# menickname/waafle

Hardware: AMD Instinct MI355X
Metric: contigs scored/sec + k2 clade-pair evals/sec at 1/2/4/8 MI355X vs CPU ref (higher is better)
Workload: dtype f64

## Files before the change

waafle_amd/csrc/wf_device.h:

```cpp
#pragma once
#include "wf_internal.h"

#include "waafle_hip.h"
#include "wf_lanes.h"

namespace wf {

namespace {


constexpr uint64_t kKeyPad = ~0ull;

#include "wf_stamps.h"
constexpr int kLocVirtual = 0xFFFF;

__device__ __forceinline__ void note_ppot(const KArgs& K, int c, int iteration, int Pp) {
  if (!K.ppot || Pp < 2) return;
  const uint64_t old = (uint64_t)K.ppot[c];
  if (iteration > (int)(old >> 40))
    K.ppot[c] = (int64_t)(((uint64_t)iteration << 40) | ((old & ((1ull << 40) - 1ull)) + (uint64_t)Pp));
}

__device__ __forceinline__ bool e2_no_option(const KArgs& K, int c, int iteration, int64_t pair_evals, bool root,
                                             int32_t* pend) {
  const int lane = threadIdx.x & 63;
  if (!root && iteration + 1 <= kMaxIter) {
    if (lane == 0) {
      pend[c] = 2;
      K.pair_evals[c] = pair_evals;
    }
    return true;
  }
  if (lane == 0) {
    K.iters[c] = (int16_t)min(root ? iteration : iteration + 1, 32767);
    K.pair_evals[c] = pair_evals;
    K.status[c] = root ? 0 : WF_E_RUNAWAY;
  }
  return false;
}

struct Ctl {
  int A, A1, npow, S_n, P, Gu, Pp;
  int overflow, status, cnt, cnt2, p_unk, root_present, all_ignored;
  int n_in, all_ok, all_same, best_ok, best_dir, best_c1p, best_c2p;
  int lca1, lca2, res_kind, lca_out;
  int cls_cnt[5], cls_off[5];
  double best_r, best_crit;
  long long best_k;
  int64_t need;
  double red_r[kWaves];
  long long red_k[kWaves];
  int red_i[kWaves];
  int red_j[kWaves];
};

__device__ __forceinline__ int lane_id() { return threadIdx.x & 63; }
__device__ __forceinline__ int wave_id() { return threadIdx.x >> 6; }

struct Arena {
  char* base;
  int64_t cap;
  int64_t used;
  template <class T>
  __device__ __forceinline__ T* take(int64_t count) {
    int64_t off = (used + 15) & ~int64_t(15);
    used = off + count * (int64_t)sizeof(T);
    return reinterpret_cast<T*>(base + off);
  }
  __device__ __forceinline__ bool fits() const { return used <= cap; }
};

__device__ __forceinline__ uint64_t dbits(double x) { return (uint64_t)__double_as_longlong(x); }

template <class T>
__device__ __forceinline__ const T& kernarg_fresh(const T& arg) {
#ifdef __HIP_DEVICE_COMPILE__
  uint64_t a = reinterpret_cast<uint64_t>(__builtin_amdgcn_kernarg_segment_ptr());
  asm volatile("" : "+s"(a));
  return *reinterpret_cast<const __attribute__((address_space(4))) T*>(a);
#else
  return arg;
#endif
}


template <int NT>
__device__ __forceinline__ int block_scan(int v, int* total, Ctl& ctl) {
  const int lane = lane_id(), w = wave_id();
  int x = v;
#pragma unroll
  for (int d = 1; d < 64; d <<= 1) {
    int y = __shfl_up(x, d, 64);
    if (lane >= d) x += y;
  }
  if (lane == 63) ctl.red_i[w] = x;
  __syncthreads();
  int base = 0, tot = 0;
#pragma unroll
  for (int i = 0; i < NT / 64; ++i) {
    int t = ctl.red_i[i];
    base += (i < w) ? t : 0;
    tot += t;
  }
  __syncthreads();
  *total = tot;
  return base + x - v;
}

template <int NT>
__device__ __forceinline__ void block_scan2(int v1, int v2, int* p1, int* p2, int* t1, int* t2, Ctl& ctl) {
  const int lane = lane_id(), w = wave_id();
  int x = v1, y = v2;
#pragma unroll
  for (int d = 1; d < 64; d <<= 1) {
    int a = __shfl_up(x, d, 64), b = __shfl_up(y, d, 64);
    if (lane >= d) { x += a; y += b; }
  }
  if (lane == 63) { ctl.red_i[w] = x; ctl.red_j[w] = y; }
  __syncthreads();
  int b1 = 0, b2 = 0, s1 = 0, s2 = 0;
#pragma unroll
  for (int i = 0; i < NT / 64; ++i) {
    int a = ctl.red_i[i], b = ctl.red_j[i];
    if (i < w) { b1 += a; b2 += b; }
    s1 += a;
    s2 += b;
  }
  __syncthreads();
  *p1 = b1 + x - v1;
  *p2 = b2 + y - v2;
  *t1 = s1;
  *t2 = s2;
}

__device__ __forceinline__ bool better(double r2, long long k2, double r, long long k) {
  return k2 >= 0 && (k < 0 || r2 > r || (r2 == r && k2 > k));
}

template <int NT>
__device__ __forceinline__ void block_argmax(double& r, long long& k, Ctl& ctl) {
#pragma unroll
  for (int off = 32; off > 0; off >>= 1) {
    double r2 = __shfl_xor(r, off, 64);
    long long k2 = __shfl_xor(k, off, 64);
    if (better(r2, k2, r, k)) { r = r2; k = k2; }
  }
  if (lane_id() == 0) { ctl.red_r[wave_id()] = r; ctl.red_k[wave_id()] = k; }
  __syncthreads();
  if (threadIdx.x == 0) {
    double br = ctl.red_r[0];
    long long bk = ctl.red_k[0];
    for (int i = 1; i < NT / 64; ++i)
      if (better(ctl.red_r[i], ctl.red_k[i], br, bk)) { br = ctl.red_r[i]; bk = ctl.red_k[i]; }
    ctl.best_r = br;
    ctl.best_k = bk;
  }
  __syncthreads();
  r = ctl.best_r;
  k = ctl.best_k;
}

template <int NT, class T>
__device__ __forceinline__ void bitonic_sort(T* keys, int n) {
  for (int k = 2; k <= n; k <<= 1) {
// ... 1674 lines not shown
```

waafle_amd/csrc/wf_fast.hip:

```cpp
#include <algorithm>
#include <cstdlib>

#include "wf_device.h"
#include "wf_lanes.h"

namespace wf {

namespace {

constexpr int kSlotBits = 9;
constexpr int kCladeShift = 15;
constexpr uint32_t kSlotMask = (1u << kSlotBits) - 1;
constexpr int kLoc0 = 64;
constexpr int kLut0 = 256;
constexpr int kAnn0 = 64;
constexpr int kRuns0 = 64;
constexpr int kMultiAtt0 = 32;
constexpr int kRunsL0 = 32;
constexpr int kMultiAttL0 = 16;
constexpr int kXcds = 8;
constexpr int kRollWaves = 4;
constexpr int kPot0 = 64;
constexpr int kS0 = 640;

// ... 446 lines not shown
    b_ok = lane_bcast(b_ok, 0); b_dir = lane_bcast(b_dir, 0);
    b_c1p = lane_bcast(b_c1p, 0); b_c2p = lane_bcast(b_c2p, 0);
    bcrit = lane_bcast(bcrit, 0);
    wave_sync();
    int n_in = 0;
    bool all_ok = true, all_same = true;
    uint64_t b1 = 0, b2 = 0;
    for (int i = 0; i + 1 < Pp; ++i) {
      const uint64_t mi = pmask[i];
      for (int j = i + 1 + lane; j < Pp; j += 64) {
        if ((mi | pmask[j]) != full) continue;
        const double r = pair_rank(C, i, j, Gu);
        if (!((br - r) <= P.range)) continue;
        const OptEval e = eval_two_call(K, C, Pn, i, j, F.best_syn(), nullptr);
        ++n_in;
        all_ok = all_ok && e.ok;
        all_same = all_same && e.same;
        b1 |= 1ull << e.c1p;
        b2 |= 1ull << e.c2p;
      }
    }
    n_in = wave_sum_dpp(n_in);
    b1 = wave_or_dpp(b1);
    b2 = wave_or_dpp(b2);
    all_ok = __ballot(!all_ok) == 0ull;
    all_same = __ballot(!all_same) == 0ull;
    int kind;
    if (n_in == 0) kind = (P.dis2 == 0) ? 3 : (P.dis2 == 1 ? 0 : 4);
    else if (n_in == 1 || P.dis2 == 0) kind = 1;
    else if (P.dis2 == 1) kind = 0;
    else kind = (all_ok && all_same) ? 2 : 0;
    if (kind == 4) {
      if (lane == 0) K.status[c] = WF_E_BADINPUT;
      return kDecDone;
    }
    bool have_ok = false;
    int lca1 = -1, lca2v = -1;
    const int m1 = __popcll(b1), m2 = __popcll(b2);
    if (kind == 2) {
      const bool in1 = lane < Pp && ((b1 >> lane) & 1ull), in2 = lane < Pp && ((b2 >> lane) & 1ull);
      lca1 = wave_lca(K, in1 ? F.cl()[lane] : -1);
      lca2v = wave_lca(K, in2 ? F.cl()[lane] : -1);
      bool keep = true;
      if (!P.allow_lca) {
        const int nl = lca2(K, lca1, lca2v);
        keep = !(nl == lca1 || nl == lca2v);
      }
      have_ok = keep;
      if (have_ok) {
        if (in1) K.meld[C.mbase + __popcll(b1 & lanes_below())] = F.cl()[lane];
        if (in2) K.meld[C.mbase + m1 + __popcll(b2 & lanes_below())] = F.cl()[lane];
      }
    } else if (kind == 1) {
      have_ok = b_ok != 0;
    } else if (kind == 3) {
      have_ok = true;
    }
    if (have_ok) {
      if (lane < G) K.syn[l0 + lane] = F.best_syn()[lane];
      if (lane == 0) {
        K.call[c] = WF_CALL_LGT;
        K.crit[c] = bcrit;
        K.rank[c] = br;
        K.dir[c] = (int8_t)b_dir;
        K.c1[c] = (kind == 2) ? lca1 : F.cl()[b_c1p];
        K.c2[c] = (kind == 2) ? lca2v : F.cl()[b_c2p];
        K.nm1[c] = (kind == 2) ? m1 : 0;
        K.nm2[c] = (kind == 2) ? m2 : 0;
        K.iters[c] = (int16_t)iteration;
        K.pair_evals[c] = pair_evals;
      }
      return kDecDone;
    }
  }
  return (Pn == 0 || root) ? kDecStop : kDecRaise;
}

template <int CAP, bool FULL, bool ROLL = false>
__global__ __launch_bounds__(64, FULL ? 2 : (ROLL ? kRollWaves : 4)) void k_wave(const SArgs S_arg, int64_t* ccnt, int64_t* cleaves, int32_t* pend,
                                             const int32_t* list, int n_list, const int64_t* n_dev, int rollup,
                                             int start_level_arg) {
  static_assert(!(FULL && ROLL), "the roll-up passes are first-form launches");
  const int start_level = ROLL ? start_level_arg : 0;
  if (n_dev) n_list = (int)*n_dev;
  if (S_arg.wq && (int)blockIdx.x >= n_list) return;
  extern __shared__ __attribute__((aligned(16))) char smem[];
  WaveSmem<CAP, FULL>& F = *reinterpret_cast<WaveSmem<CAP, FULL>*>(smem);
  const int lane = threadIdx.x;
  const bool xmap = gridDim.x % kXcds == 0;
  const int xb = (int)gridDim.x / kXcds, xj = (int)blockIdx.x / kXcds, xx = (int)blockIdx.x % kXcds;
  for (int it = 0;; ++it) {
    int ci;
    if (S_arg.wq) {
      unsigned long long q = 0;
      if (lane == 0) q = atomicAdd(S_arg.wq, 1ull);
      ci = __builtin_amdgcn_readfirstlane((int)q);
    } else {
      ci = xmap ? (it * kXcds + xx) * xb + xj : (int)blockIdx.x + it * (int)gridDim.x;
    }
    if (ci >= n_list) break;
    const int c = list ? list[ci] : ci;
    WLAP_MARK();
    const SArgs& S = kernarg_fresh<SArgs>(S_arg);
    const KArgs& K = S.k;
    const DevParams& P = K.p;
    const int nsys = K.n_sys;
    const bool ann_on = !ROLL && nsys > 0;
    if (FULL && P.weak == 2) continue;
    const int64_t h0 = K.hit_off[c], h1 = K.hit_off[c + 1];
    constexpr int kHB = 4;
    int r_qlo[kHB], r_qhi[kHB], r_hs[kHB], r_cl[kHB];
    double r_scv[kHB], r_sc[kHB];
    uint32_t r_m[kHB];
    auto load_round = [&](int64_t hq) {
#pragma unroll
      for (int b = 0; b < kHB; ++b) {
        const int64_t h = hq + 64 * b + lane;
        r_qlo[b] = 0; r_qhi[b] = 0; r_hs[b] = 0; r_cl[b] = 0;
        r_scv[b] = 0.0; r_sc[b] = 0.0; r_m[b] = 0u;
        if (h < h1) {
          r_scv[b] = K.scov[h];
          r_qlo[b] = K.qlo[h];
          r_qhi[b] = K.qhi[h];
          if (P.stranded) r_hs[b] = K.hstrand[h];
          r_cl[b] = K.taxon[h];
          r_sc[b] = K.score[h];
          if (ann_on) r_m[b] = K.sysmask[h];
        }
      }
    };
    load_round(h0);
    const int64_t l0 = K.loc_off[c];
    const int G = (int)(K.loc_off[c + 1] - l0);
    const int Gs = min(G, kLoc0);
    int nl1 = 0;
    int my_lo = 0, my_hi = -1;
    if (lane < Gs) {
      const int a = K.lstart[l0 + lane], b = K.lend[l0 + lane];
      const int len = max(a, b) - min(a, b) + 1;
      my_lo = min(a, b);
      my_hi = max(a, b);
      F.lo[lane] = my_lo;
      F.len[lane] = len;
      F.st[lane] = K.lstrand[l0 + lane];
      if (len < kNpyBuf) nl1 = S.lut_off[len + 1] - S.lut_off[len];
      F.nl1[lane] = (int16_t)nl1;
    }
    const int prev_hi = __shfl_up(my_hi, 1, 64);
    const bool ordered = G <= kLoc0 && P.min_overlap > 0.0 &&
                         __ballot(lane >= 1 && lane < Gs && my_lo <= prev_hi) == 0ull;
    int lut_total;
    const int lb = wave_excl_scan(nl1, &lut_total);
    F.lbase[lane] = (int16_t)min(lb, 32767);
    const int nann = Gs * nsys;
    F.abest()[lane] = 0ull;
    F.ahit()[lane] = -1;
    const bool long_locus = __ballot(lane < Gs && F.len[lane] > 65535) != 0ull;
    bool staged = G > kLoc0 || lut_total > kLut0 || nann > kAnn0 || long_locus;
    wave_sync();
    bool lut_ready = false;
    auto load_lut = [&]() {
      for (int i = lane; i < lut_total; i += 64) {
        int g = 0;
        for (int b = 32; b > 0; b >>= 1)
          if (g + b < Gs && F.lbase[g + b] <= i) g += b;
        F.lut[i] = pack_leaf(S.lut[S.lut_off[F.len[g]] + (i - F.lbase[g])]);
      }
      wave_sync();
      lut_ready = true;
    };

    WLAP(0);
    int n_att = 0;
    long long nl_sum = 0;
    for (int64_t hq = h0; hq < h1; hq += 64 * kHB) {
      if (hq != h0) load_round(hq);
    for (int bq = 0; bq < kHB && hq + 64 * bq < h1; ++bq) {
      const int64_t hb = hq + 64 * bq;
      const int64_t h = hb + lane;
      int qlo = r_qlo[0], qhi = r_qhi[0], hs = r_hs[0], clade = r_cl[0];
      double scv = r_scv[0], sc = r_sc[0];
      uint32_t m = r_m[0];
      int n = 0;
      uint64_t am = 0ull;
#pragma unroll
      for (int b = 1; b < kHB; ++b)
        if (bq == b) {
          qlo = r_qlo[b]; qhi = r_qhi[b]; hs = r_hs[b]; clade = r_cl[b];
          scv = r_scv[b]; sc = r_sc[b]; m = r_m[b];
        }
      if (ordered && h < h1 && scv >= P.min_scov) {
        int g = 0;
#pragma unroll
        for (int k = 32; k > 0; k >>= 1) {
          const int i = min(g + k, Gs) - 1;
          if (g + k <= Gs && F.lo[i] + F.len[i] - 1 < qlo) g += k;
        }
        for (; g < Gs; ++g) {
          const int lo = F.lo[g], len = F.len[g];
          if (lo > qhi) break;
          if (attaches(P, qlo, qhi, hs, lo, len, F.st[g])) {
            ++n;
            nl_sum += len < kNpyBuf ? F.nl1[g] : leaves_for(S, len);
            am |= 1ull << g;
          }
        }
        if (ROLL && n > 0) clade = S.anc[clade];
      } else if (!ordered && h < h1 && scv >= P.min_scov) {
        for (int g = 0; g < G; ++g) {
          int lo, len, st;
          if (g < kLoc0) {
            lo = F.lo[g]; len = F.len[g]; st = F.st[g];
          } else {
            const int a = K.lstart[l0 + g], b = K.lend[l0 + g];
            lo = min(a, b); len = max(a, b) - lo + 1; st = K.lstrand[l0 + g];
          }
          if (attaches(P, qlo, qhi, hs, lo, len, st)) {
            ++n;
            nl_sum += (g < kLoc0 && len < kNpyBuf) ? F.nl1[g] : leaves_for(S, len);
            if (g < kLoc0) am |= 1ull << g;
          }
        }
        if (ROLL && n > 0) clade = S.anc[clade];
      }
      int total;
      const int o = wave_excl_scan(n, &total);
      if (!staged && n > 0 && n_att + o + n <= CAP) {
        if (!ROLL)
          for (int j = 0; j < P.jump; ++j) clade = K.parent[clade];
        const bool ann = m != 0 && sc >= P.annot_ref;
// ... 730 lines not shown
            S.dump_cg[base + t] = cg_of(F, t);
            S.dump_mean[base + t] = out_v(t);
          }
        }
        if (lane == 0) {
          S.dump_first[slot] = (int)(base < INT32_MAX ? base : INT32_MAX);
          S.dump_first[slot + 1] = (int)(base + n_out < INT32_MAX ? base + n_out : INT32_MAX);
          S.dump_list[2 * slot] = compact ? 1 : 0;
          S.dump_list[2 * slot + 1] = dumped ? c : -1;
          if (compact) S.dump_um[slot] = um | (rootp ? (1ull << 63) : 0ull);
        }
        staged = true;
        WSTAT(21, 1);
        WLAP(9);
        break;
      }
      WLAP(9);
      if (staged || outcome == 2) break;
      const int Gu = __popcll(um);
      wave_sync();
      int dec = -1;
      if constexpr (FULL) dec = wave_two(S, F, c, h0, l0, G, ns, um, Gu, iteration, pair_evals);
      if (dec < 0) {
        staged = true;
        break;
      }
      if (dec == kDecDone) break;
      if (dec == kDecRaise && iteration + 1 <= kMaxIter) {
        if (!rollup) {
          staged = true;
          seed = iteration == 1;
          if (lane == 0) K.pair_evals[c] = pair_evals;
          break;
        }
        wave_sync();
        continue;
      }
      if (lane == 0) {
        K.iters[c] = (int16_t)min(dec == kDecRaise ? iteration + 1 : iteration, 32767);
        K.pair_evals[c] = pair_evals;
        K.status[c] = dec == kDecRaise ? WF_E_RUNAWAY : 0;
      }
      break;
    }
    if (lane == 0) {
      ccnt[c] = staged ? n_att : 0;
      cleaves[c] = staged ? nl_sum : 0;
      const int pd = staged ? (dumped ? 3 : (seed ? 2 : 1)) : 0;
      pend[c] = pd;
      if (pd == 1 && S.fail_ctr) atomicAdd(S.fail_ctr, 1ull);
    }
    WSTAT(22, staged ? 1 : 0);
    wave_sync();
    WLAP(10);
  }
}

template <int CAP, bool FULL, bool ROLL = false>
int blocks_per_cu() {
  static const int n = [] {
    const int bytes = (int)sizeof(WaveSmem<CAP, FULL>);
    (void)hipFuncSetAttribute(reinterpret_cast<const void*>(&k_wave<CAP, FULL, ROLL>),
                              hipFuncAttributeMaxDynamicSharedMemorySize, bytes);
    int b = 0;
    if (hipOccupancyMaxActiveBlocksPerMultiprocessor(&b, reinterpret_cast<const void*>(&k_wave<CAP, FULL, ROLL>), 64,
                                                     bytes) != hipSuccess || b < 1)
      b = 1;
    return b;
  }();
  return n;
}

template <int CAP, bool FULL, bool ROLL = false>
hipError_t launch_cap(const SArgs& sa, int64_t* ccnt, int64_t* cleaves, int32_t* pend, const int32_t* list,
                      int n_list, const int64_t* n_dev, int cus, int rollup, hipStream_t s, int start_level = 0) {
  const unsigned grid = (unsigned)std::max<int64_t>(1, std::min<int64_t>(n_list, (int64_t)cus * blocks_per_cu<CAP, FULL, ROLL>()));
  hipLaunchKernelGGL((k_wave<CAP, FULL, ROLL>), dim3(grid), dim3(64), sizeof(WaveSmem<CAP, FULL>), s, sa, ccnt, cleaves, pend,
                     list, n_list, n_dev, rollup, start_level);
  return hipGetLastError();
}

}

WF_STAMP_READER(fast, g_wstamps, 48)

hipError_t launch_fast(const SArgs& sa, int64_t* ccnt, int64_t* cleaves, int32_t* pend, int max_hits, int cus,
                       hipStream_t s) {
  const int N = sa.k.n_contigs;
  if (max_hits <= 224) return launch_cap<224, false>(sa, ccnt, cleaves, pend, nullptr, N, nullptr, cus, 0, s);
  return max_hits <= 256 ? launch_cap<256, false>(sa, ccnt, cleaves, pend, nullptr, N, nullptr, cus, 0, s)
                         : launch_cap<512, false>(sa, ccnt, cleaves, pend, nullptr, N, nullptr, cus, 0, s);
}

hipError_t launch_fast_list(const SArgs& sa, int64_t* ccnt, int64_t* cleaves, int32_t* pend, const int32_t* list,
                            const int64_t* n_dev, int max_hits, int cus, hipStream_t s) {
  const int N = sa.k.n_contigs;
  if (max_hits <= 224) return launch_cap<224, false>(sa, ccnt, cleaves, pend, list, N, n_dev, cus, 0, s);
  return max_hits <= 256 ? launch_cap<256, false>(sa, ccnt, cleaves, pend, list, N, n_dev, cus, 0, s)
                         : launch_cap<512, false>(sa, ccnt, cleaves, pend, list, N, n_dev, cus, 0, s);
}

hipError_t launch_level(const SArgs& sa, int64_t* ccnt, int64_t* cleaves, int32_t* pend, const int32_t* list,
                        const int64_t* n_dev, int level, int max_hits, int cus, hipStream_t s) {
  const int N = sa.k.n_contigs;
  if (max_hits <= 224) return launch_cap<224, false, true>(sa, ccnt, cleaves, pend, list, N, n_dev, cus, 0, s, level);
  return max_hits <= 256 ? launch_cap<256, false, true>(sa, ccnt, cleaves, pend, list, N, n_dev, cus, 0, s, level)
                         : launch_cap<512, false, true>(sa, ccnt, cleaves, pend, list, N, n_dev, cus, 0, s, level);
}

hipError_t launch_full(const SArgs& sa, int64_t* ccnt, int64_t* cleaves, int32_t* pend, const int32_t* list,
                       const int64_t* n_dev, int max_hits, int cus, bool rollup, hipStream_t s) {
  const int N = sa.k.n_contigs;
  return max_hits <= 256 ? launch_cap<256, true>(sa, ccnt, cleaves, pend, list, N, n_dev, cus, rollup, s)
                         : launch_cap<512, true>(sa, ccnt, cleaves, pend, list, N, n_dev, cus, rollup, s);
}

}
```

waafle_amd/csrc/wf_stamps.h:

```cpp
#pragma once
#ifdef WF_STAMPS
#ifndef WF_STAMPS_ROLL
#define WF_STAMPS_ROLL 0
#endif
#define WF_STAMPS_ONLY(...) __VA_ARGS__
#define WF_STAMP_READER(tag, arr, n)                                                          \
  extern "C" int wf_stamps_read_##tag(unsigned long long* out, int m) {                       \
    if (m > (n)) m = (n);                                                                     \
    return hipMemcpyFromSymbol(out, HIP_SYMBOL(arr), sizeof(unsigned long long) * m) == hipSuccess ? 0 : -2; \
  }                                                                                           \
  extern "C" int wf_stamps_reset_##tag(void) {                                                \
    unsigned long long z[n] = {0};                                                            \
    return hipMemcpyToSymbol(HIP_SYMBOL(arr), z, sizeof z) == hipSuccess ? 0 : -2;            \
  }
__device__ unsigned long long g_stamps[32];
__shared__ unsigned long long g_tlast;
#define STAMP_INIT() do { if (threadIdx.x == 0) g_tlast = __builtin_amdgcn_s_memtime(); } while (0)
#define STAMP(i)                                                                    \
  do {                                                                              \
    if (threadIdx.x == 0) {                                                         \
      unsigned long long now_ = __builtin_amdgcn_s_memtime();                       \
      atomicAdd(&g_stamps[i], now_ - g_tlast);                                      \
      g_tlast = now_;                                                               \
    }                                                                               \
  } while (0)
#define STAMP_SYNC() __syncthreads()
#define LAP_MARK() unsigned long long lap_ = __builtin_amdgcn_s_memtime()
#define LAP(i)                                                                      \
  do {                                                                              \
    unsigned long long n_ = __builtin_amdgcn_s_memtime();                           \
    if (threadIdx.x == 0) atomicAdd(&g_stamps[i], n_ - lap_);                       \
    lap_ = n_;                                                                      \
  } while (0)
#define LAP_WAIT_LDS() __builtin_amdgcn_s_waitcnt(0xc07f)
#define LAP_WAIT_V(v) asm volatile("" ::"v"(v))
#define STAT(i, v) do { if (threadIdx.x == 0) atomicAdd(&g_stamps[i], (unsigned long long)(v)); } while (0)
__device__ unsigned long long g_wstamps[48];
#define WLAP_MARK() unsigned long long wlap_ = __builtin_amdgcn_s_memtime(); const bool wsamp_ = !FULL && (WF_STAMPS_ROLL ? ROLL : !ROLL) && (c & 15) == 0
#define WLAP(i)                                                                     \
  do {                                                                              \
    const unsigned long long n_ = __builtin_amdgcn_s_memtime();                     \
    if (wsamp_ && lane == 0) atomicAdd(&g_wstamps[i], n_ - wlap_);                  \
    wlap_ = n_;                                                                     \
  } while (0)
#define WSTAT(i, v) do { if (wsamp_ && lane == 0) atomicAdd(&g_wstamps[i], (unsigned long long)(v)); } while (0)
__device__ unsigned long long g_tstamps[16];
#define TLAP_MARK() unsigned long long tlap_ = __builtin_amdgcn_s_memtime(); const bool tsamp_ = (c & 15) == 0
#define TLAP(i)                                                                     \
  do {                                                                              \
    const unsigned long long n_ = __builtin_amdgcn_s_memtime();                     \
    if (tsamp_ && lane == 0) atomicAdd(&g_tstamps[i], n_ - tlap_);                  \
    tlap_ = n_;                                                                     \
  } while (0)
__device__ unsigned long long g_sstamps[16];
#define SLAP_MARK(c) unsigned long long slap_ = __builtin_amdgcn_s_memtime(); const bool ssamp_ = ((c) & 7) == 0
#define SLAP(i)                                                                     \
  do {                                                                              \
    const unsigned long long n_ = __builtin_amdgcn_s_memtime();                     \
    if (ssamp_ && (threadIdx.x & 63) == 0) atomicAdd(&g_sstamps[i], n_ - slap_);    \
    slap_ = n_;                                                                     \
  } while (0)
#define SSTAT(i, v) do { if (ssamp_ && (threadIdx.x & 63) == 0) atomicAdd(&g_sstamps[i], (unsigned long long)(v)); } while (0)
__device__ unsigned long long g_bstamps[48];
#define BLAP_MARK(c) unsigned long long blap_ = __builtin_amdgcn_s_memtime(); const bool bsamp_ = ((c) & 7) == 0
#define BLAP(i)                                                                     \
  do {                                                                              \
    const unsigned long long n_ = __builtin_amdgcn_s_memtime();                     \
    if (bsamp_ && (threadIdx.x & 63) == 0) {                                        \
      atomicAdd(&g_bstamps[i], n_ - blap_);                                         \
      if (level > 0) atomicAdd(&g_bstamps[24 + (i)], n_ - blap_);                   \
    }                                                                               \
    blap_ = n_;                                                                     \
  } while (0)
#define BSTAT(i, v) do { if (bsamp_ && (threadIdx.x & 63) == 0) atomicAdd(&g_bstamps[i], (unsigned long long)(v)); } while (0)
#else
#define WF_STAMPS_ONLY(...)
#define WF_STAMP_READER(tag, arr, n)
#define STAMP_INIT() do {} while (0)
#define STAMP(i) do {} while (0)
#define STAMP_SYNC() do {} while (0)
#define LAP_MARK() do {} while (0)
#define LAP(i) do {} while (0)
#define LAP_WAIT_LDS() do {} while (0)
#define LAP_WAIT_V(v) do {} while (0)
#define STAT(i, v) do {} while (0)
#define WLAP_MARK() do {} while (0)
#define WLAP(i) do {} while (0)
#define WSTAT(i, v) do {} while (0)
#define TLAP_MARK() do {} while (0)
#define TLAP(i) do {} while (0)
#define BLAP_MARK(c) do {} while (0)
#define BLAP(i) do {} while (0)
#define BSTAT(i, v) do {} while (0)
#define SLAP_MARK(c) do {} while (0)
#define SLAP(i) do {} while (0)
#define SSTAT(i, v) do {} while (0)
#endif
```

waafle_amd/csrc/wf_triage.hip:

```cpp
#include "wf_device.h"
#include "wf_lanes.h"


namespace wf {

namespace {


constexpr int kTrHB = 4;
constexpr int kTrLoc = 64;
constexpr int kTrTab = 128;
constexpr int kTrSeg = 64;
constexpr int kTrSpan = 26;
constexpr uint32_t kTrEmpty = 0xFFFFFFFFu;
constexpr int kTrXcds = 8;
constexpr int kTrWaves = 8;
constexpr int kTrBig = 512;
constexpr int kCntR = 4;

struct TriSmem {
  int lo[kTrLoc], hi[kTrLoc];
  uint32_t tkey[kTrTab];
  uint64_t tmask[kTrTab];
  uint64_t abest[kTrLoc];
  int ahit[kTrLoc];
  int scnt[kTrSeg];
  uint32_t slohi[kTrSeg];
  uint64_t spart[kTrSeg];
  uint64_t sfw[kTrSeg];
  int fcl[kTrSeg];
  int8_t tfull[kTrTab];
  int8_t st[kTrLoc];
};
static_assert(sizeof(TriSmem) <= 160 * 1024 / (4 * kTrWaves), "triage slice: kTrWaves per SIMD");

__device__ __forceinline__ uint32_t tr_hash(uint32_t clade) { return (clade * 0x9E3779B1u) >> 25; }

__device__ __forceinline__ uint32_t tr_lohi(int qlo, int qhi, int llo, int len) {
  const int h1s = max(0, qlo - llo);
  const int h2s = min(len - 1, qhi - llo);
  const int start = min(h1s, len);
  int stop = h2s + 1;
  if (stop < 0) { stop += len; if (stop < 0) stop = 0; }
  return (uint32_t)start | ((uint32_t)stop << 16);
}


__global__ void k_pack_keys(const KArgs K, int64_t n_hits, uint32_t* key) {
  for (int64_t h = blockIdx.x * (int64_t)blockDim.x + threadIdx.x; h < n_hits; h += (int64_t)gridDim.x * blockDim.x)
    key[h] = (uint32_t)K.taxon[h] | (K.scov[h] >= K.p.min_scov ? kKeyScov : 0u) | (K.hstrand[h] == 1 ? kKeyMinus : 0u) |
             (K.n_sys > 0 ? (K.sysmask[h] & 63u) << kKeySys : 0u);
}

template <bool SYSKEY>
__global__ __launch_bounds__(64, kTrWaves) void k_triage(const SArgs S_arg, int64_t* ccnt, int64_t* cleaves,
                                                         int32_t* pend) {
  __shared__ TriSmem F;
  const int lane = threadIdx.x;
  const int N = S_arg.k.n_contigs;
  const bool xmap = gridDim.x % kTrXcds == 0;
  const int xb = (int)gridDim.x / kTrXcds, xj = (int)blockIdx.x / kTrXcds, xx = (int)blockIdx.x % kTrXcds;
  for (int it = 0;; ++it) {
    const int c = xmap ? (it * kTrXcds + xx) * xb + xj : (int)blockIdx.x + it * (int)gridDim.x;
    if (c >= N) break;
    TLAP_MARK();
    const SArgs& S = kernarg_fresh<SArgs>(S_arg);
    const KArgs& K = S.k;
    const DevParams& P = K.p;
    const int nsys = K.n_sys;
    auto hand_on = [&]() {
      if (lane == 0) pend[c] = kPendTriage;
    };
    const int64_t h0 = K.hit_off[c], h1 = K.hit_off[c + 1];
    const int64_t nh = h1 - h0;
    const int64_t hend = min(h1, h0 + 64 * kTrHB);
    int r_qlo[kTrHB], r_qhi[kTrHB];
    uint32_t r_k[kTrHB];
    double r_sc[kTrHB];
    uint32_t r_m[SYSKEY ? 1 : kTrHB];
#pragma unroll
    for (int b = 0; b < kTrHB; ++b) {
      const int64_t h = h0 + 64 * b + lane;
      r_qlo[b] = 0; r_qhi[b] = 0; r_k[b] = 0u; r_sc[b] = 0.0;
      if (!SYSKEY) r_m[b] = 0u;
      if (h < hend) {
        r_qlo[b] = K.qlo[h];
        r_qhi[b] = K.qhi[h];
        r_k[b] = K.hkey[h];
        r_sc[b] = K.score[h];
        if (!SYSKEY && nsys > 0) r_m[b] = K.sysmask[h];
      }
    }
    auto sysm = [&](int b) -> uint32_t { return SYSKEY ? r_k[b] >> kKeySys : r_m[b]; };
    const int64_t l0 = K.loc_off[c];
    const int G = (int)(K.loc_off[c + 1] - l0);
    int my_lo = 0, my_hi = -1, my_st = 0;
    if (lane < G && G <= kTrLoc) {
      const int a = K.lstart[l0 + lane], e = K.lend[l0 + lane];
      my_lo = min(a, e);
      my_hi = max(a, e);
      my_st = K.lstrand[l0 + lane];
    }
    const int prev_hi = __shfl_up(my_hi, 1, 64);
    const bool take =
        nh > 0 && nh <= 64 * kTrHB && G > 0 && G <= kTrLoc && G * nsys <= kTrLoc && P.min_overlap > 0.0 &&
        P.k1 > 0.0 && P.weak != 2 &&
        __ballot(lane < G && ((lane >= 1 && my_lo <= prev_hi) || my_hi - my_lo + 1 >= kNpyBuf)) == 0ull;
    if (!take) {
      hand_on();
      continue;
    }
    const uint64_t allG = G >= 64 ? ~0ull : ((1ull << G) - 1ull);
    const int nann = G * nsys;
    const bool ann_on = nsys > 0;
    if (lane < G) { F.lo[lane] = my_lo; F.hi[lane] = my_hi; F.st[lane] = (int8_t)my_st; }
    F.tkey[lane] = kTrEmpty; F.tkey[lane + 64] = kTrEmpty;
    F.tmask[lane] = 0ull; F.tmask[lane + 64] = 0ull;
    F.abest[lane] = 0ull; F.ahit[lane] = -1;
    F.scnt[lane] = 0; F.sfw[lane] = 0ull; F.spart[lane] = 0ull;
    wave_sync();
    TLAP(0);
    uint32_t r_am[kTrHB];
    bool bad = false;
#pragma unroll
    for (int b = 0; b < kTrHB; ++b) {
      uint32_t am = 0u;
      if (h0 + 64 * b + lane < hend && (r_k[b] & kKeyScov)) {
        const int qlo = r_qlo[b], qhi = r_qhi[b];
        int g = 0;
#pragma unroll
        for (int k = 32; k > 0; k >>= 1) {
          const int gk = g + k;
          g = (gk <= G && F.hi[min(gk, G) - 1] < qlo) ? gk : g;
        }
        const int g0 = g;
        uint32_t rel = 0u;
        for (; g < G; ++g) {
          const int lo = F.lo[g];
          if (lo > qhi) break;
          if (attaches(P, qlo, qhi, (r_k[b] & kKeyMinus) ? 1 : 0, lo, F.hi[g] - lo + 1, F.st[g])) {
            if (g - g0 < kTrSpan) rel |= 1u << (g - g0);
            else bad = true;
          }
        }
        if (rel) {
          am = (uint32_t)g0 | (rel << 6);
          int cl = (int)(r_k[b] & kKeyTaxon);
          for (int j = 0; j < P.jump; ++j) cl = K.parent[cl];
          r_k[b] = (r_k[b] & ~kKeyTaxon) | (uint32_t)cl;
        }
      }
      r_am[b] = am;
    }
    TLAP(1);
#pragma unroll
    for (int b = 0; b < kTrHB; ++b) {
      if ((r_am[b] & 0x7Fu) == 0x40u) {
        const uint32_t cl = r_k[b] & kKeyTaxon;
        uint32_t slot = tr_hash(cl);
        for (int probes = 0;; ++probes) {
          if (probes == kTrTab) { bad = true; break; }
          const uint32_t old = atomicCAS(&F.tkey[slot], kTrEmpty, cl);
          if (old == kTrEmpty || old == cl) break;
          slot = (slot + 1) & (kTrTab - 1);
        }
      }
    }
    if (__ballot(bad) != 0ull) {
      hand_on();
      wave_sync();
      continue;
    }
    wave_sync();
    TLAP(2);
#pragma unroll
    for (int b = 0; b < kTrHB; ++b) {
      const uint32_t am = r_am[b];
      int found = -1;
      if (am != 0u) {
        const int g0 = (int)(am & 63u);
        const uint64_t lm = (uint64_t)(am >> 6) << g0;
        const uint32_t cl = r_k[b] & kKeyTaxon;
        uint32_t slot = tr_hash(cl);
        for (int probes = 0; probes < kTrTab; ++probes) {
          const uint32_t k = F.tkey[slot];
          if (k == cl) { atomicOr(&F.tmask[slot], lm); found = (int)slot; break; }
          if (k == kTrEmpty) break;
          slot = (slot + 1) & (kTrTab - 1);
        }
        const uint32_t m = sysm(b);
        if (ann_on && m != 0u && r_sc[b] >= P.annot_ref)
          for (uint64_t bits = lm; bits; bits &= bits - 1) {
            const int g = __builtin_ctzll(bits);
            for (int s = 0; s < nsys; ++s)
              if ((m >> s) & 1u) atomicMax(&F.abest[g * nsys + s], dbits(r_sc[b]));
          }
      }
      r_k[b] = (r_k[b] & ~kKeyTaxon) | (uint32_t)(found + 1);
    }
    wave_sync();
    TLAP(3);
    int nfull = 0;
#pragma unroll
    for (int half = 0; half < 2; ++half) {
      const int e = lane + 64 * half;
      const bool full = F.tkey[e] != kTrEmpty && F.tmask[e] == allG;
      const uint64_t fm = __ballot(full);
      const int fi = nfull + __popcll(fm & ((1ull << lane) - 1ull));
      F.tfull[e] = (int8_t)(full && fi * G < kTrSeg ? fi : -1);
      if (full && fi * G < kTrSeg) F.fcl[fi] = (int)F.tkey[e];
      nfull += __popcll(fm);
    }
    if (nfull == 0 || nfull * G > kTrSeg) {
      hand_on();
      wave_sync();
      continue;
    }
    wave_sync();
    TLAP(4);
#pragma unroll
    for (int b = 0; b < kTrHB; ++b) {
      const uint32_t am = r_am[b];
      int fi = -1;
      if (am != 0u) {
        const int g0 = (int)(am & 63u);
        const int slot = (int)(r_k[b] & kKeyTaxon) - 1;
        fi = slot >= 0 ? (int)F.tfull[slot] : -1;
        if (fi >= 0)
          for (uint32_t rel = am >> 6; rel; rel &= rel - 1) {
            const int g = g0 + __builtin_ctz(rel);
            const int q = fi * G + g;
            const int llo = F.lo[g], len = F.hi[g] - llo + 1;
            const uint32_t lh = tr_lohi(r_qlo[b], r_qhi[b], llo, len);
            atomicAdd(&F.scnt[q], 1);
            F.slohi[q] = lh;
            const int lo = (int)(lh & 0xFFFFu), hi = (int)(lh >> 16);
            if (lo < hi) atomicMax(&F.spart[q], dbits(r_sc[b]));
            if (lo <= 0 && hi >= len && r_sc[b] > 0.0) atomicMax(&F.sfw[q], dbits(r_sc[b]));
          }
        const uint32_t m = sysm(b);
        if (ann_on && m != 0u && r_sc[b] >= P.annot_ref) {
          const int h = (int)(h0 + 64 * b + lane);
          for (uint64_t bits = (uint64_t)(am >> 6) << g0; bits; bits &= bits - 1) {
            const int g = __builtin_ctzll(bits);
            for (int s = 0; s < nsys; ++s)
              if (((m >> s) & 1u) && F.abest[g * nsys + s] == dbits(r_sc[b])) atomicMax(&F.ahit[g * nsys + s], h);
          }
        }
      }
    }
    wave_sync();
    TLAP(5);
    const int nseg = nfull * G;
    const int my_g = lane % G, my_f = lane / G;
    double mean = 0.0;
    bool fail = false;
    if (lane < nseg) {
      const int n = F.scnt[lane];
      const int len = F.hi[my_g] - F.lo[my_g] + 1;
      int lo = 0, hi = len;
      double v = 0.0;
      const double vp = __longlong_as_double((long long)F.spart[lane]);
      const double vw = __longlong_as_double((long long)F.sfw[lane]);
      if (n == 1) {
        const uint32_t lh = F.slohi[lane];
        lo = (int)(lh & 0xFFFFu); hi = (int)(lh >> 16); v = vp;
      } else if (!(vp > vw)) {
        v = vw;
      } else {
        fail = true;
      }
      hi = max(hi, lo);
      const double sum = (lo <= 0 && hi >= len) ? pw_const_sum(len, v) : pw_run_sum(len, lo, hi, v);
      mean = (0.0 + sum) / (double)len;
    }
    TLAP(6);
    const bool sure_l = lane < nseg && F.fcl[my_f] != K.unknown && mean >= P.kmin;
    const uint64_t sure = wave_or_dpp(sure_l ? 1ull << my_g : 0ull);
    const bool um_all = P.weak != 0 || P.kmin <= 0.0;
    if (__ballot(fail) != 0ull || (!um_all && sure != allG)) {
      hand_on();
      wave_sync();
      continue;
    }
    double my_r = -__builtin_inf(), my_c = 0.0;
    for (int i = 0; i < nfull; ++i) {
      const int base = i * G;
      const int m8 = G < 8 ? 0 : G - (G & 7);
      double r0 = 0.0, r1 = 0.0, r2 = 0.0, r3 = 0.0, r4 = 0.0, r5 = 0.0, r6 = 0.0, r7 = 0.0;
      double mn = __builtin_inf();
      for (int u = 0; u < m8; u += 8) {
        const double x0 = lane_bcast(mean, base + u), x1 = lane_bcast(mean, base + u + 1);
        const double x2 = lane_bcast(mean, base + u + 2), x3 = lane_bcast(mean, base + u + 3);
        const double x4 = lane_bcast(mean, base + u + 4), x5 = lane_bcast(mean, base + u + 5);
        const double x6 = lane_bcast(mean, base + u + 6), x7 = lane_bcast(mean, base + u + 7);
        r0 += x0; r1 += x1; r2 += x2; r3 += x3; r4 += x4; r5 += x5; r6 += x6; r7 += x7;
        mn = x0 < mn ? x0 : mn; mn = x1 < mn ? x1 : mn; mn = x2 < mn ? x2 : mn; mn = x3 < mn ? x3 : mn;
        mn = x4 < mn ? x4 : mn; mn = x5 < mn ? x5 : mn; mn = x6 < mn ? x6 : mn; mn = x7 < mn ? x7 : mn;
      }
      double res = m8 > 0 ? leaf_tree(r0, r1, r2, r3, r4, r5, r6, r7) : 0.0;
      for (int u = m8; u < G; ++u) {
        const double x = lane_bcast(mean, base + u);
        mn = x < mn ? x : mn;
        res += x;
      }
      if (lane == i) { my_r = (0.0 + res) / (double)G; my_c = mn; }
    }
    TLAP(7);
    const bool mine = lane < nfull;
    const int my_cl = mine ? F.fcl[lane] : -1;
    const bool opt = mine && my_c >= P.k1;
    double br = opt ? my_r : -__builtin_inf(), bcrit = opt ? my_c : 0.0;
    long long bk = opt ? my_cl : -1;
    each_stride([&](auto J) {
      const double r2 = xor_lanes<decltype(J)::value>(br), c2 = xor_lanes<decltype(J)::value>(bcrit);
      const long long k2 = xor_lanes<decltype(J)::value>(bk);
      if (better(r2, k2, br, bk)) { br = r2; bk = k2; bcrit = c2; }
    });
    if (bk < 0) {
      hand_on();
      wave_sync();
      continue;
    }
    int nm = 0, lca = (int)bk;
    const bool in = P.dis1 == 1 && opt && (br - my_r) <= P.range;
    const uint64_t inm = __ballot(in);
    if (P.dis1 == 1) {
      nm = __popcll(inm);
      if (nm == 0) {
        hand_on();
        wave_sync();
        continue;
      }
      if (nm > 1) {
        int acc = in ? my_cl : -1;
        each_stride([&](auto J) { acc = lca2(K, acc, xor_lanes<decltype(J)::value>(acc)); });
        lca = acc;
      }
      int pos = 0;
      for (uint64_t rest = inm; rest; rest &= rest - 1) pos += lane_bcast(my_cl, __builtin_ctzll(rest)) < my_cl ? 1 : 0;
      if (in) K.meld[2 * h0 + 2 * (int64_t)c + pos] = my_cl;
    }
    if (lane < G) K.syn[l0 + lane] = 'A';
    if (ann_on && lane < nann) K.annot[l0 * nsys + lane] = F.ahit[lane];
    if (lane == 0) {
      K.call[c] = WF_CALL_NO_LGT;
      K.crit[c] = bcrit;
      K.rank[c] = br;
      K.c1[c] = lca;
      K.c2[c] = -1;
      K.nm1[c] = nm;
      K.iters[c] = 1;
      K.pair_evals[c] = 0;
      ccnt[c] = 0;
      cleaves[c] = 0;
      pend[c] = 0;
    }
    wave_sync();
    TLAP(8);
    WF_STAMPS_ONLY(if (tsamp_ && lane == 0) atomicAdd(&g_tstamps[15], 1ull));
  }
}

__global__ __launch_bounds__(64) void k_count(const SArgs S, int64_t* ccnt, int64_t* cleaves, int32_t* pend) {
  __shared__ int s_lo[kTrLoc], s_hi[kTrLoc], s_nl[kTrLoc];
  __shared__ int8_t s_st[kTrLoc];
  const KArgs& K = S.k;
  const DevParams& P = K.p;
  const int lane = threadIdx.x;
  unsigned long long n_staged = 0;
  auto leaves = [&](int len) {
    return (len / kNpyBuf) * (S.lut_off[kNpyBuf + 1] - S.lut_off[kNpyBuf]) +
           (S.lut_off[len % kNpyBuf + 1] - S.lut_off[len % kNpyBuf]);
  };
  for (int c = blockIdx.x; c < K.n_contigs; c += gridDim.x) {
    const int64_t h0 = K.hit_off[c], h1 = K.hit_off[c + 1];
    if (h1 - h0 <= kTrBig) continue;
    const int64_t l0 = K.loc_off[c];
    const int G = (int)(K.loc_off[c + 1] - l0);
    int clo = 0, chi = -1, cst = 0;
    if (lane < G && G <= kTrLoc) {
      const int a = K.lstart[l0 + lane], e = K.lend[l0 + lane];
      clo = min(a, e);
      chi = max(a, e);
      cst = K.lstrand[l0 + lane];
    }
    const int cprev = __shfl_up(chi, 1, 64);
    if (!(G > 0 && G <= kTrLoc && P.min_overlap > 0.0 && __ballot(lane < G && lane >= 1 && clo <= cprev) == 0ull))
      continue;
    if (lane < G) { s_lo[lane] = clo; s_hi[lane] = chi; s_st[lane] = (int8_t)cst; s_nl[lane] = leaves(chi - clo + 1); }
    wave_sync();
    long long n_att = 0, nl = 0;
    for (int64_t hb = h0; hb < h1; hb += 64 * kCntR) {
      uint32_t r_k[kCntR];
      int r_qlo[kCntR], r_qhi[kCntR];
#pragma unroll
      for (int r = 0; r < kCntR; ++r) {
        const int64_t h = hb + 64 * r + lane;
        r_k[r] = 0u; r_qlo[r] = 0; r_qhi[r] = 0;
        if (h < h1) { r_k[r] = K.hkey[h]; r_qlo[r] = K.qlo[h]; r_qhi[r] = K.qhi[h]; }
      }
#pragma unroll
      for (int r = 0; r < kCntR; ++r) {
        if (hb + 64 * r + lane >= h1 || !(r_k[r] & kKeyScov)) continue;
        const int qlo = r_qlo[r], qhi = r_qhi[r], hs = (r_k[r] & kKeyMinus) ? 1 : 0;
        int g = 0;
#pragma unroll
        for (int k = 32; k > 0; k >>= 1)
          if (g + k <= G && s_hi[g + k - 1] < qlo) g += k;
        for (; g < G; ++g) {
          const int lo = s_lo[g];
          if (lo > qhi) break;
          const int len = s_hi[g] - lo + 1;
          if (attaches(P, qlo, qhi, hs, lo, len, s_st[g])) {
            ++n_att;
            nl += s_nl[g];
          }
        }
      }
    }
    n_att = wave_sum_dpp(n_att);
    nl = wave_sum_dpp(nl);
    if (lane == 0) {
      ccnt[c] = n_att;
      cleaves[c] = nl;
      pend[c] = 1;
    }
    ++n_staged;
    wave_sync();
  }
  if (lane == 0 && n_staged && S.fail_ctr) atomicAdd(S.fail_ctr, n_staged);
}


}

WF_STAMP_READER(triage, g_tstamps, 16)

template <bool SYSKEY>
int triage_per_cu() {
  static const int per_cu = [] {
    int b = 0;
    if (hipOccupancyMaxActiveBlocksPerMultiprocessor(&b, reinterpret_cast<const void*>(&k_triage<SYSKEY>), 64, 0) !=
            hipSuccess || b < 1)
      b = 1;
    return b;
  }();
  return per_cu;
}

hipError_t pack_keys(const KArgs& k, int64_t n_hits, uint32_t* key, int cus, hipStream_t s) {
  if (n_hits > 0)
    hipLaunchKernelGGL(k_pack_keys, dim3((unsigned)std::min<int64_t>((n_hits + 255) / 256, (int64_t)cus * 16)),
                       dim3(256), 0, s, k, n_hits, key);
  return hipGetLastError();
}

hipError_t launch_triage(const SArgs& sa, int64_t* ccnt, int64_t* cleaves, int32_t* pend, int max_hits, int cus,
                         hipStream_t s) {
  const int N = sa.k.n_contigs;
  if (sa.k.n_sys <= 6) {
    const unsigned grid = (unsigned)std::max<int64_t>(1, std::min<int64_t>(N, (int64_t)cus * triage_per_cu<true>()));
// ... 13 lines not shown
```

Before: 116.3 million.

## Prefetch next contig's offsets via scalar loads and hoist locus loads

Per-contig hit and locus offsets are now read through scalar-cache (constant address space) loads, and in the static schedule the next contig's offsets are fetched one iteration ahead, so the head of each iteration no longer waits on dependent global loads. Locus start/end/strand loads are issued before the hit-register round, and the LUT lookups are reordered to overlap with them. The same read-ahead is applied to the triage kernel, and k_count switches to scalar loads. Timing sub-stamps are also added but compile out by default. The cost is extra live registers and reliance on the offset arrays being safe to read through the scalar cache.

```diff
diff --git a/waafle_amd/csrc/wf_device.h b/waafle_amd/csrc/wf_device.h
--- a/waafle_amd/csrc/wf_device.h
+++ b/waafle_amd/csrc/wf_device.h
@@ -80,6 +80,15 @@
   return *reinterpret_cast<const __attribute__((address_space(4))) T*>(a);
 #else
   return arg;
+#endif
+}
+
+template <class T>
+__device__ __forceinline__ T uniform_load(const T* p) {
+#ifdef __HIP_DEVICE_COMPILE__
+  return *reinterpret_cast<const __attribute__((address_space(4))) T*>(reinterpret_cast<uint64_t>(p));
+#else
+  return *p;
 #endif
 }
 
diff --git a/waafle_amd/csrc/wf_fast.hip b/waafle_amd/csrc/wf_fast.hip
--- a/waafle_amd/csrc/wf_fast.hip
+++ b/waafle_amd/csrc/wf_fast.hip
@@ -552,32 +552,61 @@
                                              int start_level_arg) {
   static_assert(!(FULL && ROLL), "the roll-up passes are first-form launches");
   const int start_level = ROLL ? start_level_arg : 0;
-  if (n_dev) n_list = (int)*n_dev;
+  if (n_dev) n_list = (int)uniform_load(n_dev);
   if (S_arg.wq && (int)blockIdx.x >= n_list) return;
   extern __shared__ __attribute__((aligned(16))) char smem[];
   WaveSmem<CAP, FULL>& F = *reinterpret_cast<WaveSmem<CAP, FULL>*>(smem);
   const int lane = threadIdx.x;
   const bool xmap = gridDim.x % kXcds == 0;
   const int xb = (int)gridDim.x / kXcds, xj = (int)blockIdx.x / kXcds, xx = (int)blockIdx.x % kXcds;
+  auto contig_at = [&](int it) {
+    return xmap ? (it * kXcds + xx) * xb + xj : (int)blockIdx.x + it * (int)gridDim.x;
+  };
+  int nx_c = 0, nx_G = 0;
+  int64_t nx_h0 = 0, nx_h1 = 0, nx_l0 = 0;
+  auto read_offsets = [&](const KArgs& K, int ci_n) {
+    const int cn = list ? uniform_load(list + ci_n) : ci_n;
+    const int64_t a = uniform_load(K.hit_off + cn), b = uniform_load(K.hit_off + cn + 1);
+    const int64_t l = uniform_load(K.loc_off + cn), m = uniform_load(K.loc_off + cn + 1);
+    nx_c = cn; nx_h0 = a; nx_h1 = b; nx_l0 = l; nx_G = (int)(m - l);
+  };
+  if (!S_arg.wq && contig_at(0) < n_list) read_offsets(S_arg.k, contig_at(0));
   for (int it = 0;; ++it) {
     int ci;
+    WF_STAMPS_ONLY(const unsigned long long wq0_ = __builtin_amdgcn_s_memtime());
     if (S_arg.wq) {
       unsigned long long q = 0;
       if (lane == 0) q = atomicAdd(S_arg.wq, 1ull);
       ci = __builtin_amdgcn_readfirstlane((int)q);
     } else {
-      ci = xmap ? (it * kXcds + xx) * xb + xj : (int)blockIdx.x + it * (int)gridDim.x;
+      ci = contig_at(it);
     }
     if (ci >= n_list) break;
-    const int c = list ? list[ci] : ci;
+    WF_STAMPS_ONLY(const unsigned long long wq1_ = __builtin_amdgcn_s_memtime());
+    if (S_arg.wq) read_offsets(S_arg.k, ci);
+    const int c = nx_c;
+    const int64_t h0 = nx_h0, h1 = nx_h1, l0 = nx_l0;
+    const int G = nx_G;
+    if (!S_arg.wq && contig_at(it + 1) < n_list) read_offsets(S_arg.k, contig_at(it + 1));
+    HEAD_WAIT_S(c);
     WLAP_MARK();
+    WSTAT(48, wq1_ - wq0_);
+    WSTAT(49, wlap_ - wq1_);
     const SArgs& S = kernarg_fresh<SArgs>(S_arg);
     const KArgs& K = S.k;
     const DevParams& P = K.p;
     const int nsys = K.n_sys;
     const bool ann_on = !ROLL && nsys > 0;
     if (FULL && P.weak == 2) continue;
-    const int64_t h0 = K.hit_off[c], h1 = K.hit_off[c + 1];
+    HEAD_WAIT_S(h0); HEAD_WAIT_S(h1); HEAD_WAIT_S(l0); HEAD_WAIT_S(G);
+    WSUB(50);
+    const int Gs = min(G, kLoc0);
+    int loc_a = 0, loc_b = 0, loc_st = 0;
+    if (lane < Gs) {
+      loc_a = K.lstart[l0 + lane];
+      loc_b = K.lend[l0 + lane];
+      loc_st = K.lstrand[l0 + lane];
+    }
     constexpr int kHB = 4;
     int r_qlo[kHB], r_qhi[kHB], r_hs[kHB], r_cl[kHB];
     double r_scv[kHB], r_sc[kHB];
@@ -599,23 +628,26 @@
         }
       }
     };
-    load_round(h0);
-    const int64_t l0 = K.loc_off[c];
-    const int G = (int)(K.loc_off[c + 1] - l0);
-    const int Gs = min(G, kLoc0);
     int nl1 = 0;
-    int my_lo = 0, my_hi = -1;
+    int my_lo = 0, my_hi = -1, my_len = kNpyBuf;
     if (lane < Gs) {
-      const int a = K.lstart[l0 + lane], b = K.lend[l0 + lane];
-      const int len = max(a, b) - min(a, b) + 1;
+      const int a = loc_a, b = loc_b;
+      my_len = max(a, b) - min(a, b) + 1;
       my_lo = min(a, b);
       my_hi = max(a, b);
       F.lo[lane] = my_lo;
-      F.len[lane] = len;
-      F.st[lane] = K.lstrand[l0 + lane];
-      if (len < kNpyBuf) nl1 = S.lut_off[len + 1] - S.lut_off[len];
-      F.nl1[lane] = (int16_t)nl1;
-    }
+      F.len[lane] = my_len;
+      F.st[lane] = loc_st;
+    }
+    HEAD_WAIT_V(my_lo); HEAD_WAIT_V(my_hi);
+    WSUB(51);
+    int lut_a = 0, lut_b = 0;
+    if (lane < Gs && my_len < kNpyBuf) { lut_a = S.lut_off[my_len]; lut_b = S.lut_off[my_len + 1]; }
+    load_round(h0);
+    nl1 = lut_b - lut_a;
+    if (lane < Gs) F.nl1[lane] = (int16_t)nl1;
+    HEAD_WAIT_V(nl1);
+    WSUB(52);
     const int prev_hi = __shfl_up(my_hi, 1, 64);
     const bool ordered = G <= kLoc0 && P.min_overlap > 0.0 &&
                          __ballot(lane >= 1 && lane < Gs && my_lo <= prev_hi) == 0ull;
@@ -1512,7 +1544,7 @@
 
 }
 
-WF_STAMP_READER(fast, g_wstamps, 48)
+WF_STAMP_READER(fast, g_wstamps, 56)
 
 hipError_t launch_fast(const SArgs& sa, int64_t* ccnt, int64_t* cleaves, int32_t* pend, int max_hits, int cus,
                        hipStream_t s) {
diff --git a/waafle_amd/csrc/wf_stamps.h b/waafle_amd/csrc/wf_stamps.h
--- a/waafle_amd/csrc/wf_stamps.h
+++ b/waafle_amd/csrc/wf_stamps.h
@@ -35,8 +35,8 @@
 #define LAP_WAIT_LDS() __builtin_amdgcn_s_waitcnt(0xc07f)
 #define LAP_WAIT_V(v) asm volatile("" ::"v"(v))
 #define STAT(i, v) do { if (threadIdx.x == 0) atomicAdd(&g_stamps[i], (unsigned long long)(v)); } while (0)
-__device__ unsigned long long g_wstamps[48];
-#define WLAP_MARK() unsigned long long wlap_ = __builtin_amdgcn_s_memtime(); const bool wsamp_ = !FULL && (WF_STAMPS_ROLL ? ROLL : !ROLL) && (c & 15) == 0
+__device__ unsigned long long g_wstamps[56];
+#define WLAP_MARK() unsigned long long wlap_ = __builtin_amdgcn_s_memtime(), wsub_ = wlap_; const bool wsamp_ = !FULL && (WF_STAMPS_ROLL ? ROLL : !ROLL) && (c & 15) == 0
 #define WLAP(i)                                                                     \
   do {                                                                              \
     const unsigned long long n_ = __builtin_amdgcn_s_memtime();                     \
@@ -45,13 +45,27 @@
   } while (0)
 #define WSTAT(i, v) do { if (wsamp_ && lane == 0) atomicAdd(&g_wstamps[i], (unsigned long long)(v)); } while (0)
 __device__ unsigned long long g_tstamps[16];
-#define TLAP_MARK() unsigned long long tlap_ = __builtin_amdgcn_s_memtime(); const bool tsamp_ = (c & 15) == 0
+#define TLAP_MARK() unsigned long long tlap_ = __builtin_amdgcn_s_memtime(), tsub_ = tlap_; const bool tsamp_ = (c & 15) == 0
 #define TLAP(i)                                                                     \
   do {                                                                              \
     const unsigned long long n_ = __builtin_amdgcn_s_memtime();                     \
     if (tsamp_ && lane == 0) atomicAdd(&g_tstamps[i], n_ - tlap_);                  \
     tlap_ = n_;                                                                     \
   } while (0)
+#define TSUB(i)                                                                     \
+  do {                                                                              \
+    const unsigned long long n_ = __builtin_amdgcn_s_memtime();                     \
+    if (tsamp_ && lane == 0) atomicAdd(&g_tstamps[i], n_ - tsub_);                  \
+    tsub_ = n_;                                                                     \
+  } while (0)
+#define WSUB(i)                                                                     \
+  do {                                                                              \
+    const unsigned long long n_ = __builtin_amdgcn_s_memtime();                     \
+    if (wsamp_ && lane == 0) atomicAdd(&g_wstamps[i], n_ - wsub_);                  \
+    wsub_ = n_;                                                                     \
+  } while (0)
+#define HEAD_WAIT_S(x) asm volatile("" ::"s"(x))
+#define HEAD_WAIT_V(x) asm volatile("" ::"v"(x))
 __device__ unsigned long long g_sstamps[16];
 #define SLAP_MARK(c) unsigned long long slap_ = __builtin_amdgcn_s_memtime(); const bool ssamp_ = ((c) & 7) == 0
 #define SLAP(i)                                                                     \
@@ -89,6 +103,10 @@
 #define WSTAT(i, v) do {} while (0)
 #define TLAP_MARK() do {} while (0)
 #define TLAP(i) do {} while (0)
+#define TSUB(i) do {} while (0)
+#define WSUB(i) do {} while (0)
+#define HEAD_WAIT_S(x) do {} while (0)
+#define HEAD_WAIT_V(x) do {} while (0)
 #define BLAP_MARK(c) do {} while (0)
 #define BLAP(i) do {} while (0)
 #define BSTAT(i, v) do {} while (0)
diff --git a/waafle_amd/csrc/wf_triage.hip b/waafle_amd/csrc/wf_triage.hip
--- a/waafle_amd/csrc/wf_triage.hip
+++ b/waafle_amd/csrc/wf_triage.hip
@@ -60,8 +60,20 @@
   const int N = S_arg.k.n_contigs;
   const bool xmap = gridDim.x % kTrXcds == 0;
   const int xb = (int)gridDim.x / kTrXcds, xj = (int)blockIdx.x / kTrXcds, xx = (int)blockIdx.x % kTrXcds;
+  auto contig_at = [&](int it) {
+    return xmap ? (it * kTrXcds + xx) * xb + xj : (int)blockIdx.x + it * (int)gridDim.x;
+  };
+  int64_t nx_h0 = 0, nx_l0 = 0;
+  int nx_nh = 0, nx_G = 0;
+  auto read_ahead = [&](const KArgs& K, int cn) {
+    const int64_t a = uniform_load(K.hit_off + cn), b = uniform_load(K.hit_off + cn + 1);
+    const int64_t l = uniform_load(K.loc_off + cn), m = uniform_load(K.loc_off + cn + 1);
+    nx_h0 = a; nx_nh = (int)(b - a);
+    nx_l0 = l; nx_G = (int)(m - l);
+  };
+  if (contig_at(0) < N) read_ahead(S_arg.k, contig_at(0));
   for (int it = 0;; ++it) {
-    const int c = xmap ? (it * kTrXcds + xx) * xb + xj : (int)blockIdx.x + it * (int)gridDim.x;
+    const int c = contig_at(it);
     if (c >= N) break;
     TLAP_MARK();
     const SArgs& S = kernarg_fresh<SArgs>(S_arg);
@@ -71,9 +83,22 @@
     auto hand_on = [&]() {
       if (lane == 0) pend[c] = kPendTriage;
     };
-    const int64_t h0 = K.hit_off[c], h1 = K.hit_off[c + 1];
-    const int64_t nh = h1 - h0;
-    const int64_t hend = min(h1, h0 + 64 * kTrHB);
+    const int64_t h0 = nx_h0, l0 = nx_l0;
+    const int nh = nx_nh, G = nx_G;
+    const int64_t hend = h0 + min(nh, 64 * kTrHB);
+    HEAD_WAIT_S(h0); HEAD_WAIT_S(nh); HEAD_WAIT_S(l0); HEAD_WAIT_S(G);
+    TSUB(9);
+    const bool has_locus = lane < G && G <= kTrLoc;
+    int loc_a = 0, loc_e = -1, my_st = 0;
+    if (has_locus) {
+      loc_a = K.lstart[l0 + lane];
+      loc_e = K.lend[l0 + lane];
+      my_st = K.lstrand[l0 + lane];
+    }
+    const int32_t* const f_qlo = K.qlo;
+    const int32_t* const f_qhi = K.qhi;
+    const uint32_t* const f_key = K.hkey;
+    const double* const f_sc = K.score;
     int r_qlo[kTrHB], r_qhi[kTrHB];
     uint32_t r_k[kTrHB];
     double r_sc[kTrHB];
@@ -84,29 +109,32 @@
       r_qlo[b] = 0; r_qhi[b] = 0; r_k[b] = 0u; r_sc[b] = 0.0;
       if (!SYSKEY) r_m[b] = 0u;
       if (h < hend) {
-        r_qlo[b] = K.qlo[h];
-        r_qhi[b] = K.qhi[h];
-        r_k[b] = K.hkey[h];
-        r_sc[b] = K.score[h];
+        r_qlo[b] = f_qlo[h];
+        r_qhi[b] = f_qhi[h];
+        r_k[b] = f_key[h];
+        r_sc[b] = f_sc[h];
         if (!SYSKEY && nsys > 0) r_m[b] = K.sysmask[h];
       }
     }
     auto sysm = [&](int b) -> uint32_t { return SYSKEY ? r_k[b] >> kKeySys : r_m[b]; };
-    const int64_t l0 = K.loc_off[c];
-    const int G = (int)(K.loc_off[c + 1] - l0);
-    int my_lo = 0, my_hi = -1, my_st = 0;
-    if (lane < G && G <= kTrLoc) {
-      const int a = K.lstart[l0 + lane], e = K.lend[l0 + lane];
-      my_lo = min(a, e);
-      my_hi = max(a, e);
-      my_st = K.lstrand[l0 + lane];
-    }
+    auto settle_loads = [&]() {
+      asm volatile("" ::"v"(my_st), "v"(r_sc[kTrHB - 1]), "v"(r_m[SYSKEY ? 0 : kTrHB - 1]));
+    };
+    {
+      const int cn = contig_at(it + 1);
+      if (cn < N) read_ahead(K, cn);
+    }
+    TSUB(10);
+    const int my_lo = has_locus ? min(loc_a, loc_e) : 0, my_hi = has_locus ? max(loc_a, loc_e) : -1;
+    HEAD_WAIT_V(my_lo); HEAD_WAIT_V(my_hi); HEAD_WAIT_V(my_st);
+    TSUB(11);
     const int prev_hi = __shfl_up(my_hi, 1, 64);
     const bool take =
         nh > 0 && nh <= 64 * kTrHB && G > 0 && G <= kTrLoc && G * nsys <= kTrLoc && P.min_overlap > 0.0 &&
         P.k1 > 0.0 && P.weak != 2 &&
         __ballot(lane < G && ((lane >= 1 && my_lo <= prev_hi) || my_hi - my_lo + 1 >= kNpyBuf)) == 0ull;
     if (!take) {
+      settle_loads();
       hand_on();
       continue;
     }
@@ -114,11 +142,16 @@
     const int nann = G * nsys;
     const bool ann_on = nsys > 0;
     if (lane < G) { F.lo[lane] = my_lo; F.hi[lane] = my_hi; F.st[lane] = (int8_t)my_st; }
+    asm volatile("" ::"v"(my_st));
     F.tkey[lane] = kTrEmpty; F.tkey[lane + 64] = kTrEmpty;
     F.tmask[lane] = 0ull; F.tmask[lane + 64] = 0ull;
     F.abest[lane] = 0ull; F.ahit[lane] = -1;
     F.scnt[lane] = 0; F.sfw[lane] = 0ull; F.spart[lane] = 0ull;
     wave_sync();
+    TSUB(12);
+#pragma unroll
+    for (int b = 0; b < kTrHB; ++b) { HEAD_WAIT_V(r_qlo[b]); HEAD_WAIT_V(r_qhi[b]); HEAD_WAIT_V(r_k[b]); HEAD_WAIT_V(r_sc[b]); }
+    TSUB(13);
     TLAP(0);
     uint32_t r_am[kTrHB];
     bool bad = false;
@@ -167,6 +200,7 @@
       }
     }
     if (__ballot(bad) != 0ull) {
+      settle_loads();
       hand_on();
       wave_sync();
       continue;
@@ -212,6 +246,7 @@
       nfull += __popcll(fm);
     }
     if (nfull == 0 || nfull * G > kTrSeg) {
+      settle_loads();
       hand_on();
       wave_sync();
       continue;
@@ -374,10 +409,10 @@
            (S.lut_off[len % kNpyBuf + 1] - S.lut_off[len % kNpyBuf]);
   };
   for (int c = blockIdx.x; c < K.n_contigs; c += gridDim.x) {
-    const int64_t h0 = K.hit_off[c], h1 = K.hit_off[c + 1];
+    const int64_t h0 = uniform_load(K.hit_off + c), h1 = uniform_load(K.hit_off + c + 1);
     if (h1 - h0 <= kTrBig) continue;
-    const int64_t l0 = K.loc_off[c];
-    const int G = (int)(K.loc_off[c + 1] - l0);
+    const int64_t l0 = uniform_load(K.loc_off + c);
+    const int G = (int)(uniform_load(K.loc_off + c + 1) - l0);
     int clo = 0, chi = -1, cst = 0;
     if (lane < G && G <= kTrLoc) {
       const int a = K.lstart[l0 + lane], e = K.lend[l0 + lane];
```

Result: no change. 117.2 million (median of 6 runs) (+0.7%).
